# johanngerberding/voxelnet-pytorch

Hardware: AMD Instinct MI355X
Metric: point-clouds/sec fwd+bwd, KITTI car voxel grid, batch=2 (higher is better)
Workload: dtype bf16; 1 GPU; KITTI car config (voxel 0.2x0.2x0.4 m, grid 10x400x352, T=35), batch=2 per GPU, fwd+bwd train step (BASELINE configs[1]); global_batch=2, points_per_frame=19861, parallelism=dp1, launch_mode=eager+native-executor+one-call-step

## Files before the change

voxelnet-pytorch_amd/csrc/wgrad.hip:

```cpp
#include "common.h"

namespace {

constexpr uint32_t WG_OOB = 0xFFFFF000u;
constexpr uint32_t WG_MAX_WINDOW = 0xFFFFE000u;

struct WGParams {
    const char *src;
    const char *rows;
    float *dw;
    int64_t sB, sD, sH, sW;
    int64_t rB, rD, rH, rW;
    int32_t B, Ds, Hs, Ws, Dr, Hr, Wr;
    int32_t mulD, mulH, mulW, tmulD, tmulH, tmulW, padD, padH, padW;
    int32_t kD, kH, kW;
    int32_t C, N;
    int32_t x3;
    int32_t rows_per_chunk;
    int32_t tiles_k;
    uint32_t src_bytes, rows_bytes;
    const int64_t *row_list;
    int64_t n_rows;
    const int32_t *row_count;
    int32_t divD, divH, divW;
    float *part;
    int64_t part_stride;
};

typedef __attribute__((address_space(3))) void lds_void_t;
typedef __attribute__((ext_vector_type(4))) short s16x4_t;
typedef __attribute__((ext_vector_type(8))) short s16x8_t;

__device__ __forceinline__ void lds_dma16(__amdgpu_buffer_rsrc_t rsrc, char *lds_wave_base, uint32_t voffset,
                                          uint32_t soffset) {
    __builtin_amdgcn_raw_ptr_buffer_load_lds(rsrc, (lds_void_t *)lds_wave_base, 16, voffset, soffset, 0, 0);
}

template <int ROW_BYTES, bool F32, bool PS = false>
__device__ __forceinline__ int chunk_swz(int row) {
    if (PS) return (row & 1) | (((row >> 1) & 1) << 2) | (((row >> 3) & 1) << 3);
    if (F32) return (row & 3) << 2;
    if (ROW_BYTES == 128) return (((row >> 1) & 1) << 1) | (((row >> 3) & 1) << 2);
    return ((row & 3) << 1) | (((row >> 3) & 1) << 3);
}

template <int TN, int TK, bool F32, int TPB, int WKW = 2, bool PS = false>
__global__ void __launch_bounds__(128 * WKW, 2) k_wgrad(const WGParams p) {
    static_assert(!PS || F32, "split storage is fp32-sized");
    constexpr int NWV = 2 * WKW;
    constexpr int ESZ = F32 ? 4 : 2;
    constexpr int ROWS = F32 ? 32 : 64;
    constexpr int DN = 32 * TN, DK = 16 * WKW * TK;
    constexpr int RBN = DN * ESZ, RBK = DK * ESZ;
    constexpr int TILE_N = ROWS * RBN, TILE_K = ROWS * RBK;
    constexpr int STAGE = TILE_N + TPB * TILE_K;
    constexpr int IN = TILE_N / (1024 * NWV), IK = TILE_K / (1024 * NWV);
    static_assert(TILE_N % (1024 * NWV) == 0 && TILE_K % (1024 * NWV) == 0, "tile bytes per stage must split over the waves");
    constexpr int LPR_N = RBN / 16, LPR_K = RBK / 16;
    constexpr int TW = TPB + 1;
    extern __shared__ __attribute__((aligned(16))) char smem[];
    uint32_t *tbl = reinterpret_cast<uint32_t *>(smem + 2 * STAGE);

    const int lane = threadIdx.x & 63;
    const int wave = __builtin_amdgcn_readfirstlane(threadIdx.x >> 6);
    const int wn = wave / WKW, wk = wave % WKW;
    const int bx = blockIdx.x, by = blockIdx.y, tile = blockIdx.z, gx = gridDim.x;
    const int tn = tile / p.tiles_k, tk = tile - tn * p.tiles_k;
    const int n0 = tn * DN, k0 = tk * DK;
    const int tap0 = by * TPB;
    const int td = tap0 / (p.kH * p.kW), th = (tap0 / p.kW) % p.kH, tw0 = tap0 % p.kW;
    const bool list = p.row_list != nullptr;
    int64_t M = list ? p.n_rows : (int64_t)p.B * p.Dr * p.Hr * p.Wr;
    if (list && p.row_count) {
        const int64_t cnt = (int64_t)p.row_count[0];
        M = cnt < 0 ? 0 : (cnt < M ? cnt : M);
    }
    const bool dealt = list && p.row_count;
    int64_t rbeg = (int64_t)bx * p.rows_per_chunk;
    if (rbeg >= M && !dealt) return;
    int64_t rend = rbeg + p.rows_per_chunk;
    if (rend > M) rend = M;
    if (rend < rbeg) rend = rbeg;
    int nsteps = (int)((rend - rbeg + ROWS - 1) / ROWS);
    int64_t slab_stride = ROWS;
    if (dealt) {
        const int64_t nslabs = (M + ROWS - 1) / ROWS;
        nsteps = (int)(nslabs > bx ? (nslabs - bx + gx - 1) / gx : 0);
        rbeg = (int64_t)bx * ROWS;
        rend = M;
        slab_stride = (int64_t)gx * ROWS;
    }
    const int nstages = nsteps;

    const __amdgpu_buffer_rsrc_t rs_s = vn_uniform_rsrc(p.src, p.src_bytes);
    const __amdgpu_buffer_rsrc_t rs_r = vn_uniform_rsrc(p.rows, p.rows_bytes);

    int cb = 0, cd = 0, ch = 0, cw = 0;
    int cm32 = lane;
    const int rows_in_chunk = (int)(rend - rbeg);
    int tstep = 0;
    const uint32_t rBb = (uint32_t)(p.rB * ESZ), rDb = (uint32_t)(p.rD * ESZ), rHb = (uint32_t)(p.rH * ESZ), rWb = (uint32_t)(p.rW * ESZ);
    const uint32_t sBb = (uint32_t)(p.sB * ESZ), sDb = (uint32_t)(p.sD * ESZ), sHb = (uint32_t)(p.sH * ESZ), sWb = (uint32_t)(p.sW * ESZ);
    if (wave == 0 && !list) {
        int64_t t = rbeg + lane;
        cw = (int)(t % p.Wr); t /= p.Wr;
        ch = (int)(t % p.Hr); t /= p.Hr;
        cd = (int)(t % p.Dr);
        cb = (int)(t / p.Dr);
    }
    auto table_write = [&](int stage_idx) {
        const int step = stage_idx;
        uint32_t so[TPB], ro = WG_OOB;
#pragma unroll
        for (int j = 0; j < TPB; ++j) so[j] = WG_OOB;
        if (list) {
            const int64_t m = rbeg + (int64_t)step * slab_stride + lane;
            if (m < rend && lane < ROWS) {
                const int64_t *rc = p.row_list + m * 4;
                const int b = (int)rc[0];
                int sd = (int)rc[1] * p.mulD + td * p.tmulD - p.padD;
                int sh = (int)rc[2] * p.mulH + th * p.tmulH - p.padH;
                ro = (uint32_t)(m * p.rW * ESZ);
                const bool dh_ok = sd >= 0 && sh >= 0 && sd % p.divD == 0 && sh % p.divH == 0;
                sd /= p.divD; sh /= p.divH;
#pragma unroll
                for (int j = 0; j < TPB; ++j) {
                    int sw = (int)rc[3] * p.mulW + (tw0 + j) * p.tmulW - p.padW;
                    const bool ok = dh_ok && sw >= 0 && sw % p.divW == 0;
                    sw /= p.divW;
                    if (ok && sd < p.Ds && sh < p.Hs && sw < p.Ws)
                        so[j] = (uint32_t)(((int64_t)b * p.sB + (int64_t)sd * p.sD + (int64_t)sh * p.sH + (int64_t)sw * p.sW) * ESZ);
                }
            }
        } else {
            while (tstep < step) {
                cm32 += ROWS;
                cw += ROWS;
#pragma unroll
                for (int k = 0; k < 3; ++k) {
                    const bool wrap = cw >= p.Wr;
                    cw -= wrap ? p.Wr : 0;
                    ch += wrap ? 1 : 0;
                }
                while (cw >= p.Wr) { cw -= p.Wr; ++ch; }
                while (ch >= p.Hr) { ch -= p.Hr; ++cd; }
                while (cd >= p.Dr) { cd -= p.Dr; ++cb; }
                ++tstep;
            }
            if (cm32 < rows_in_chunk) {
                const int sd = cd * p.mulD + td * p.tmulD - p.padD;
                const int sh = ch * p.mulH + th * p.tmulH - p.padH;
                ro = (uint32_t)cb * rBb + (uint32_t)cd * rDb + (uint32_t)ch * rHb + (uint32_t)cw * rWb;
                if ((unsigned)sd < (unsigned)p.Ds && (unsigned)sh < (unsigned)p.Hs) {
                    const uint32_t base = (uint32_t)cb * sBb + (uint32_t)sd * sDb + (uint32_t)sh * sHb;
#pragma unroll
                    for (int j = 0; j < TPB; ++j) {
                        const int sw = cw * p.mulW + (tw0 + j) * p.tmulW - p.padW;
                        if ((unsigned)sw < (unsigned)p.Ws) so[j] = base + (uint32_t)sw * sWb;
                    }
                }
            }
        }
        uint32_t *e = tbl + ((stage_idx & 1) * 64 + lane) * TW;
#pragma unroll
        for (int j = 0; j < TPB; ++j) e[j] = so[j];
        e[TPB] = ro;
    };

    auto stage = [&](int sidx, int buf) {
        const uint32_t s_col = __builtin_amdgcn_readfirstlane((uint32_t)(k0 * ESZ));
        const uint32_t r_col = __builtin_amdgcn_readfirstlane((uint32_t)(n0 * ESZ));
        const uint32_t *t = tbl + (sidx & 1) * 64 * TW;
        char *ln = smem + buf * STAGE + wave * 1024;
#pragma unroll
        for (int i = 0; i < IN; ++i) {
            const int r = ((i * NWV + wave) * 1024) / RBN + lane / LPR_N;
            const int c = (lane % LPR_N) ^ chunk_swz<RBN, F32, PS>(r);
            const uint32_t ro = t[r * TW + TPB];
            const bool ok = ro != WG_OOB && (n0 + c * (16 / ESZ)) < p.N;
            lds_dma16(rs_r, ln + i * (1024 * NWV), ok ? ro + (uint32_t)c * 16u : WG_OOB, r_col);
        }
#pragma unroll
        for (int j = 0; j < TPB; ++j) {
            char *lk = smem + buf * STAGE + TILE_N + j * TILE_K + wave * 1024;
#pragma unroll
            for (int i = 0; i < IK; ++i) {
                const int r = ((i * NWV + wave) * 1024) / RBK + lane / LPR_K;
                const int c = (lane % LPR_K) ^ chunk_swz<RBK, F32, PS>(r);
                const uint32_t so = t[r * TW + j];
                const bool ok = so != WG_OOB && (k0 + c * (16 / ESZ)) < p.C;
                lds_dma16(rs_s, lk + i * (1024 * NWV), ok ? so + (uint32_t)c * 16u : WG_OOB, s_col);
            }
        }
    };

    f32x4_t acc[TPB][TN][TK];
#pragma unroll
    for (int t = 0; t < TPB; ++t)
#pragma unroll
        for (int i = 0; i < TN; ++i)
#pragma unroll
            for (int j = 0; j < TK; ++j) acc[t][i][j] = f32x4_t{0.f, 0.f, 0.f, 0.f};

    const int g = lane >> 4, q = (lane >> 2) & 3, pp = lane & 3;

    if (wave == 0 && nstages > 0) table_write(0);
    __syncthreads();
    if (nstages > 0) stage(0, 0);
    if (wave == 0 && nstages > 1) table_write(1);
    for (int s = 0; s < nstages; ++s) {
        const int buf = s & 1;
        asm volatile("s_waitcnt vmcnt(0)" ::: "memory");
        __syncthreads();
        if (s + 1 < nstages) stage(s + 1, buf ^ 1);
        if (wave == 0 && s + 2 < nstages) table_write(s + 2);
        const char *ln = smem + buf * STAGE;
        const char *lk0 = smem + buf * STAGE + TILE_N;
        if constexpr (PS) {
            typedef __attribute__((address_space(3))) s16x4_t lds_s16x4_t;
            static_assert(ROWS == 32, "one 32-site MFMA per stage");
            const int r0 = g * 8 + q, r1 = r0 + 4;
            const int sw0 = chunk_swz<RBN, true, true>(r0), sw1 = chunk_swz<RBN, true, true>(r1);
            const int pc = (pp >> 1) * 2, ph = (pp & 1) * 8;
            auto frag = [&](const char *tile, int row_bytes, int t16, int lo) {
                const int c16 = t16 * 4 + pc + lo;
                const char *p0 = tile + r0 * row_bytes + ((c16 ^ sw0) << 4) + ph;
                const char *p1 = tile + r1 * row_bytes + ((c16 ^ sw1) << 4) + ph;
                const s16x4_t v0 = __builtin_amdgcn_ds_read_tr16_b64_v4i16((lds_s16x4_t *)p0);
                const s16x4_t v1 = __builtin_amdgcn_ds_read_tr16_b64_v4i16((lds_s16x4_t *)p1);
                const s16x8_t t8 = __builtin_shufflevector(v0, v1, 0, 1, 2, 3, 4, 5, 6, 7);
                return __builtin_bit_cast(bf16x8_t, t8);
            };
            bf16x8_t ah[TN], al[TN];
#pragma unroll
            for (int i = 0; i < TN; ++i) {
                ah[i] = frag(ln, RBN, wn * TN + i, 0);
                al[i] = frag(ln, RBN, wn * TN + i, 1);
            }
#pragma unroll
            for (int t = 0; t < TPB; ++t)
#pragma unroll
                for (int j = 0; j < TK; ++j) {
                    const bf16x8_t bh = frag(lk0 + t * TILE_K, RBK, wk * TK + j, 0);
                    const bf16x8_t bl = frag(lk0 + t * TILE_K, RBK, wk * TK + j, 1);
#pragma unroll
                    for (int i = 0; i < TN; ++i) acc[t][i][j] = vn_mfma_x3(ah[i], al[i], bh, bl, acc[t][i][j]);
                }
        } else if constexpr (F32) {
            const int fc = lane & 15, kq = lane >> 4;
            if (p.x3) {
                static_assert(ROWS == 32, "eight sites per lane");
                bf16x8_t ah[TN], al[TN];
#pragma unroll
                for (int i = 0; i < TN; ++i) {
                    const int col = (wn * TN + i) * 16 + fc;
                    float v[8];
#pragma unroll
                    for (int ss = 0; ss < 8; ++ss) {
                        const int r = ss * 4 + kq;
                        v[ss] = *reinterpret_cast<const float *>(ln + r * RBN + ((((col >> 2) ^ chunk_swz<RBN, true>(r))) << 4) + (col & 3) * 4);
                    }
                    vn_split8(v, ah[i], al[i]);
                }
#pragma unroll
                for (int t = 0; t < TPB; ++t)
#pragma unroll
                    for (int j = 0; j < TK; ++j) {
                        const int col = (wk * TK + j) * 16 + fc;
                        float v[8];
#pragma unroll
                        for (int ss = 0; ss < 8; ++ss) {
                            const int r = ss * 4 + kq;
                            v[ss] = *reinterpret_cast<const float *>(lk0 + t * TILE_K + r * RBK + ((((col >> 2) ^ chunk_swz<RBK, true>(r))) << 4) + (col & 3) * 4);
                        }
                        bf16x8_t bh, bl;
                        vn_split8(v, bh, bl);
#pragma unroll
                        for (int i = 0; i < TN; ++i) acc[t][i][j] = vn_mfma_x3(ah[i], al[i], bh, bl, acc[t][i][j]);
                    }
            } else
#pragma unroll
            for (int ss = 0; ss < ROWS / 4; ++ss) {
                const int r = ss * 4 + kq;
                const int sw = chunk_swz<RBN, true>(r);
                float a[TN];
#pragma unroll
                for (int i = 0; i < TN; ++i) {
                    const int col = (wn * TN + i) * 16 + fc;
                    a[i] = *reinterpret_cast<const float *>(ln + r * RBN + ((((col >> 2) ^ sw)) << 4) + (col & 3) * 4);
                }
#pragma unroll
                for (int t = 0; t < TPB; ++t) {
                    float b[TK];
#pragma unroll
                    for (int j = 0; j < TK; ++j) {
                        const int col = (wk * TK + j) * 16 + fc;
                        b[j] = *reinterpret_cast<const float *>(lk0 + t * TILE_K + r * RBK + ((((col >> 2) ^ sw)) << 4) + (col & 3) * 4);
                    }
#pragma unroll
                    for (int i = 0; i < TN; ++i)
#pragma unroll
                        for (int j = 0; j < TK; ++j)
                            acc[t][i][j] = __builtin_amdgcn_mfma_f32_16x16x4f32(a[i], b[j], acc[t][i][j], 0, 0, 0);
                }
            }
        } else {
            typedef __attribute__((address_space(3))) s16x4_t lds_s16x4_t;
#pragma unroll
            for (int ks = 0; ks < 2; ++ks) {
                const int r0 = ks * 32 + g * 8 + q, r1 = r0 + 4;
                bf16x8_t a[TN];
#pragma unroll
                for (int i = 0; i < TN; ++i) {
                    const int col = (wn * TN + i) * 16 + pp * 4;
                    const int c16 = col >> 3, half = (col >> 2) & 1;
                    const char *p0 = ln + r0 * RBN + ((c16 ^ chunk_swz<RBN, false>(r0)) << 4) + half * 8;
                    const char *p1 = ln + r1 * RBN + ((c16 ^ chunk_swz<RBN, false>(r1)) << 4) + half * 8;
                    const s16x4_t lo = __builtin_amdgcn_ds_read_tr16_b64_v4i16((lds_s16x4_t *)p0);
                    const s16x4_t hi = __builtin_amdgcn_ds_read_tr16_b64_v4i16((lds_s16x4_t *)p1);
                    const s16x8_t t8 = __builtin_shufflevector(lo, hi, 0, 1, 2, 3, 4, 5, 6, 7);
                    a[i] = __builtin_bit_cast(bf16x8_t, t8);
                }
#pragma unroll
                for (int t = 0; t < TPB; ++t) {
                    bf16x8_t b[TK];
#pragma unroll
                    for (int j = 0; j < TK; ++j) {
                        const int col = (wk * TK + j) * 16 + pp * 4;
                        const int c16 = col >> 3, half = (col >> 2) & 1;
                        const char *p0 = lk0 + t * TILE_K + r0 * RBK + ((c16 ^ chunk_swz<RBK, false>(r0)) << 4) + half * 8;
                        const char *p1 = lk0 + t * TILE_K + r1 * RBK + ((c16 ^ chunk_swz<RBK, false>(r1)) << 4) + half * 8;
                        const s16x4_t lo = __builtin_amdgcn_ds_read_tr16_b64_v4i16((lds_s16x4_t *)p0);
                        const s16x4_t hi = __builtin_amdgcn_ds_read_tr16_b64_v4i16((lds_s16x4_t *)p1);
                        const s16x8_t t8 = __builtin_shufflevector(lo, hi, 0, 1, 2, 3, 4, 5, 6, 7);
                        b[j] = __builtin_bit_cast(bf16x8_t, t8);
                    }
#pragma unroll
                    for (int i = 0; i < TN; ++i)
#pragma unroll
                        for (int j = 0; j < TK; ++j)
                            acc[t][i][j] = __builtin_amdgcn_mfma_f32_16x16x32_bf16(a[i], b[j], acc[t][i][j], 0, 0, 0);
                }
            }
        }
    }

    float *dst = p.part ? p.part + (int64_t)bx * p.part_stride : p.dw;
#pragma unroll
    for (int t = 0; t < TPB; ++t)
#pragma unroll
        for (int i = 0; i < TN; ++i)
#pragma unroll
            for (int j = 0; j < TK; ++j) {
                const int k = k0 + (wk * TK + j) * 16 + (lane & 15);
#pragma unroll
                for (int e = 0; e < 4; ++e) {
                    const int n = n0 + (wn * TN + i) * 16 + (lane >> 4) * 4 + e;
                    if (n < p.N && k < p.C) {
                        float *q = dst + ((int64_t)(tap0 + t) * p.N + n) * p.C + k;
                        *q = p.part ? acc[t][i][j][e] : *q + acc[t][i][j][e];
                    }
                }
            }
}

__global__ void __launch_bounds__(256) k_wgrad_reduce(const float *__restrict__ part, int chunks, int64_t n4,
                                                      float *__restrict__ dw) {
    for (int64_t i = (int64_t)blockIdx.x * 256 + threadIdx.x; i < n4; i += (int64_t)gridDim.x * 256) {
        float4 s = make_float4(0.f, 0.f, 0.f, 0.f);
        for (int c = 0; c < chunks; ++c) {
            const float4 v = reinterpret_cast<const float4 *>(part)[(int64_t)c * n4 + i];
            s.x += v.x; s.y += v.y; s.z += v.z; s.w += v.w;
        }
        float4 d = reinterpret_cast<float4 *>(dw)[i];
        d.x += s.x; d.y += s.y; d.z += s.z; d.w += s.w;
        reinterpret_cast<float4 *>(dw)[i] = d;
    }
}

struct WPParams {
    const char *src, *rows;
    float *part;
    int64_t part_stride;
    int64_t sB, sD, sH, sW, rB, rD, rH, rW;
    int32_t B, Ds, Hs, Ws, Dr, Hr, Wr;
    int32_t mulD, padD, kD;
    int32_t C, N, tiles_k;
    int32_t tiles_x, tiles_y;
    int32_t tiles_per_chunk;
    uint32_t src_bytes, rows_bytes;
    uint32_t s_cb, s_part, r_cb, r_part;
};

template <int NH>
__global__ void __launch_bounds__(256 * NH, 2) k_wgrad_patch(const WPParams p) {
    constexpr int NWV = 4 * NH;
    constexpr int TH = 4, TW = 16, PH = TH + 2, LP = 32;
    constexpr int RB = 128;
    constexpr int RBN = 128 * NH;
    constexpr int TILE_N = 64 * RBN;
    constexpr int PATCH = PH * LP * RB;
    constexpr int STAGE = TILE_N + PATCH;
    constexpr int IN = TILE_N / (1024 * NWV);
    constexpr int RPI = 1024 / RBN, LPR = RBN / 16;
    constexpr int NPP = PH * 3;
    extern __shared__ __attribute__((aligned(16))) char smem[];
    const int lane = threadIdx.x & 63;
    const int wave = __builtin_amdgcn_readfirstlane(threadIdx.x >> 6);
    const int wn = wave >> 2, wk = wave & 3;
    const int tile = blockIdx.z;
    const int tn = tile / p.tiles_k, tk = tile - tn * p.tiles_k;
    const int n0 = tn * 64 * NH, k0 = tk * 64;
    const int kd = blockIdx.y;
    const int64_t ntiles = (int64_t)p.B * p.Dr * p.tiles_y * p.tiles_x;
    const int64_t tbeg = (int64_t)blockIdx.x * p.tiles_per_chunk;
    int64_t tend = tbeg + p.tiles_per_chunk;
    if (tend > ntiles) tend = ntiles;
    const int nst = (int)(tend - tbeg);

    const __amdgpu_buffer_rsrc_t rs_s = vn_uniform_rsrc(p.src, p.src_bytes);
    const __amdgpu_buffer_rsrc_t rs_r = vn_uniform_rsrc(p.rows, p.rows_bytes);
    const uint32_t s_col = (uint32_t)(k0 >> 3) * p.s_cb + p.s_part, r_col = (uint32_t)(n0 >> 3) * p.r_cb + p.r_part;

    int r_py[IN], r_px[IN];
    uint32_t r_dlt[IN], r_chunk[IN];
#pragma unroll
    for (int i = 0; i < IN; ++i) {
        const int r = (i * NWV + wave) * RPI + lane / LPR;
        const int c = (lane % LPR) ^ chunk_swz<RBN, false>(r);
        r_py[i] = r >> 4; r_px[i] = r & 15;
        r_dlt[i] = (uint32_t)((((int64_t)(r >> 4)) * p.rH + (int64_t)(r & 15) * p.rW) * 2) + (uint32_t)c * p.r_cb;
        r_chunk[i] = (n0 + c * 8) < p.N ? 1u : 0u;
    }
    constexpr int IPP = (NPP + NWV - 1) / NWV;
    int s_qy[IPP], s_qx[IPP];
    int32_t s_dlt[IPP];
    uint32_t s_ok[IPP], s_lds[IPP];
#pragma unroll
    for (int i = 0; i < IPP; ++i) {
        const int piece = i * NWV + wave;
        const int ql = piece / 3, cg = piece - ql * 3;
        const int qx = cg * 8 + lane / 8;
        const int prow = ql * LP + qx;
        const int c = (lane % 8) ^ chunk_swz<RB, false>(prow);
        s_qy[i] = ql - 1; s_qx[i] = qx - 1;
        s_dlt[i] = (int32_t)((((int64_t)(ql - 1)) * p.sH + (int64_t)(qx - 1) * p.sW) * 2) + c * (int32_t)p.s_cb;
        s_ok[i] = (piece < NPP && qx < TW + 2 && (k0 + c * 8) < p.C) ? 1u : 0u;
        s_lds[i] = (uint32_t)((ql * LP + cg * 8) * RB);
    }
    int tx, ty, td, tb;
    {
        int64_t t = tbeg;
        tx = (int)(t % p.tiles_x); t /= p.tiles_x;
        ty = (int)(t % p.tiles_y); t /= p.tiles_y;
        td = (int)(t % p.Dr);
        tb = (int)(t / p.Dr);
    }
    auto stage = [&](int buf) {
        const int y0 = ty * TH, x0 = tx * TW;
        const int sd = td * p.mulD + kd - p.padD;
        const bool plane_ok = (unsigned)sd < (unsigned)p.Ds;
        const uint32_t rbase = (uint32_t)(((int64_t)tb * p.rB + (int64_t)td * p.rD + (int64_t)y0 * p.rH + (int64_t)x0 * p.rW) * 2);
        const uint32_t sbase = (uint32_t)(((int64_t)tb * p.sB + (int64_t)sd * p.sD + (int64_t)y0 * p.sH + (int64_t)x0 * p.sW) * 2);
        char *ln = smem + buf * STAGE + wave * 1024;
#pragma unroll
        for (int i = 0; i < IN; ++i) {
            const bool ok = plane_ok && r_chunk[i] && y0 + r_py[i] < p.Hr && x0 + r_px[i] < p.Wr;
            lds_dma16(rs_r, ln + i * (1024 * NWV), ok ? rbase + r_dlt[i] : WG_OOB, r_col);
        }
        char *lp = smem + buf * STAGE + TILE_N;
#pragma unroll
        for (int i = 0; i < IPP; ++i) {
            if (i * NWV + wave >= NPP) break;
            const bool ok = plane_ok && s_ok[i] && (unsigned)(y0 + s_qy[i]) < (unsigned)p.Hs &&
                            (unsigned)(x0 + s_qx[i]) < (unsigned)p.Ws;
            lds_dma16(rs_s, lp + s_lds[i], ok ? sbase + (uint32_t)s_dlt[i] : WG_OOB, s_col);
        }
        if (++tx == p.tiles_x) {
            tx = 0;
            if (++ty == p.tiles_y) {
                ty = 0;
                if (++td == p.Dr) { td = 0; ++tb; }
            }
        }
    };

    f32x4_t acc[9][4];
#pragma unroll
    for (int t = 0; t < 9; ++t)
#pragma unroll
        for (int i = 0; i < 4; ++i) acc[t][i] = f32x4_t{0.f, 0.f, 0.f, 0.f};

    const int g = lane >> 4, q = (lane >> 2) & 3, pp = lane & 3;
    typedef __attribute__((address_space(3))) s16x4_t lds_s16x4_t;
    int aoff[4][2];
#pragma unroll
    for (int i = 0; i < 4; ++i) {
        const int col = (wn * 4 + i) * 16 + pp * 4, c16 = col >> 3, half = (col >> 2) & 1;
        const int r0 = g * 8 + q;
        aoff[i][0] = r0 * RBN + ((c16 ^ chunk_swz<RBN, false>(r0)) << 4) + half * 8;
        aoff[i][1] = (r0 + 4) * RBN + ((c16 ^ chunk_swz<RBN, false>(r0 + 4)) << 4) + half * 8;
    }
    int boff[3][2];
#pragma unroll
    for (int tw = 0; tw < 3; ++tw)
#pragma unroll
        for (int wq = 0; wq < 2; ++wq) {
            const int colw = (g & 1) * 8 + q + tw + 4 * wq;
            const int sw = chunk_swz<RB, false>(colw);
            const int col = wk * 16 + pp * 4, c16 = col >> 3, half = (col >> 2) & 1;
            boff[tw][wq] = ((g >> 1) * LP + colw) * RB + ((c16 ^ sw) << 4) + half * 8;
        }

    stage(0);
    for (int s = 0; s < nst; ++s) {
        const int buf = s & 1;
        asm volatile("s_waitcnt vmcnt(0)" ::: "memory");
        __syncthreads();
        if (s + 1 < nst) stage(buf ^ 1);
        const char *ln = smem + buf * STAGE;
        const char *lp = ln + TILE_N;
#pragma unroll
        for (int ks = 0; ks < 2; ++ks) {
            bf16x8_t a[4];
#pragma unroll
            for (int i = 0; i < 4; ++i) {
                const s16x4_t lo = __builtin_amdgcn_ds_read_tr16_b64_v4i16((lds_s16x4_t *)(ln + ks * 32 * RBN + aoff[i][0]));
                const s16x4_t hi = __builtin_amdgcn_ds_read_tr16_b64_v4i16((lds_s16x4_t *)(ln + ks * 32 * RBN + aoff[i][1]));
                a[i] = __builtin_bit_cast(bf16x8_t, __builtin_shufflevector(lo, hi, 0, 1, 2, 3, 4, 5, 6, 7));
            }
#pragma unroll
            for (int t = 0; t < 9; ++t) {
                const int th = t / 3, tw = t % 3;
                const char *lt = lp + (ks * 2 + th) * LP * RB;
                const s16x4_t lo = __builtin_amdgcn_ds_read_tr16_b64_v4i16((lds_s16x4_t *)(lt + boff[tw][0]));
                const s16x4_t hi = __builtin_amdgcn_ds_read_tr16_b64_v4i16((lds_s16x4_t *)(lt + boff[tw][1]));
                const bf16x8_t bq = __builtin_bit_cast(bf16x8_t, __builtin_shufflevector(lo, hi, 0, 1, 2, 3, 4, 5, 6, 7));
#pragma unroll
                for (int i = 0; i < 4; ++i) acc[t][i] = __builtin_amdgcn_mfma_f32_16x16x32_bf16(bq, a[i], acc[t][i], 0, 0, 0);
            }
        }
    }
    float *dst = p.part + (int64_t)blockIdx.x * p.part_stride;
#pragma unroll
    for (int t = 0; t < 9; ++t)
#pragma unroll
        for (int i = 0; i < 4; ++i) {
            const int k = k0 + wk * 16 + (lane >> 4) * 4;
            const int n = n0 + (wn * 4 + i) * 16 + (lane & 15);
            if (n < p.N && k < p.C)
                *reinterpret_cast<f32x4_t *>(dst + ((int64_t)(kd * 9 + t) * p.N + n) * p.C + k) = acc[t][i];
        }
}

template <int TN, int TK, bool F32, int TPB, int WKW = 2, bool PS = false>
int launch_wgrad(const WGParams &p, dim3 grid, hipStream_t st) {
    constexpr int DN = 32 * TN, DK = 16 * WKW * TK;
    constexpr size_t lds = 2u * 64u * (DN + TPB * DK) * 2u + 2u * 64u * (TPB + 1) * 4u;
    static const hipError_t attr = hipFuncSetAttribute(reinterpret_cast<const void *>(&k_wgrad<TN, TK, F32, TPB, WKW, PS>),
                                                       hipFuncAttributeMaxDynamicSharedMemorySize, (int)lds);
    if (attr != hipSuccess) return (int)attr;
    k_wgrad<TN, TK, F32, TPB, WKW, PS><<<grid, 128 * WKW, lds, st>>>(p);
    VN_LAUNCH_STATUS();
    return VN_OK;
}

}

static int wgrad_impl(const void *src, const void *rows, float *dw_packed, const vnConv *g, int32_t split,
                      const int64_t *row_list, int64_t n_rows, void *workspace, size_t workspace_bytes, vnStream stream,
                      int32_t *chunks_out = nullptr, const int32_t *row_count = nullptr, int split_pass = -1);

struct WGPlan {
    bool tri, n128, k128;
    int tiles_n, tiles_k, groups;
    int64_t chunks;
    int64_t dw_elems;
};
static WGPlan wgrad_plan(const vnConv *g, int32_t split, int64_t M) {
    WGPlan w{};
    const bool f32 = g->dtype != VN_BF16;
    const int taps = g->kD * g->kH * g->kW;
    w.tri = !f32 && !split && g->kW == 3 && g->Cr <= 64;
    w.n128 = !w.tri && g->Cr > 64;
    w.k128 = g->Cs > 64;
    w.tiles_n = (int)vn_ceil_div(g->Cr, w.n128 ? 128 : 64);
    w.tiles_k = (int)vn_ceil_div(g->Cs, w.k128 ? 128 : 64);
    w.groups = w.tri ? taps / 3 : taps;
    w.dw_elems = (int64_t)taps * g->Cr * g->Cs;
    static const int knob = vn_knob("VN_WG_BLOCKS", 0);
    const int target = knob > 0 ? knob : ((g->dtype == VN_F32X3 || g->dtype == VN_F32X3S) ? 384 : 256);
    int64_t chunks = target / ((int64_t)w.groups * w.tiles_n * w.tiles_k);
    const int64_t slabs = vn_ceil_div(M, 64);
    if (chunks > slabs / 10) chunks = slabs / 10;
    if (chunks > 256) chunks = 256;
    if (chunks < 1) chunks = 1;
    w.chunks = chunks;
    return w;
}

struct WPPlan {
    bool ok;
    int nh;
    int tiles_x, tiles_y, tiles_n, tiles_k;
    int64_t ntiles, chunks;
};
static int wgrad_patch_enabled() {
    static const int v = vn_knob("VN_WGRAD_PATCH", 1);
    return v;
}
static WPPlan wgrad_patch_plan(const vnConv *g, int32_t split, bool list) {
    WPPlan w{};
    if (!wgrad_patch_enabled() || list || split || g->dtype != VN_BF16) return w;
    if (g->kH != 3 || g->kW != 3 || g->mulH != 1 || g->mulW != 1 || g->tmulH != 1 || g->tmulW != 1 || g->padH != 1 ||
        g->padW != 1 || g->tmulD != 1 || g->divD != 1 || g->divH != 1 || g->divW != 1)
        return w;
    if (g->Hs != g->Hr || g->Ws != g->Wr) return w;
    if (g->Cr > 64 || g->Hr < 128 || g->Wr < 128 || g->Cs > 64) return w;
    w.nh = 1;
    w.tiles_x = (int)vn_ceil_div(g->Wr, 16);
    w.tiles_y = (int)vn_ceil_div(g->Hr, 4);
    w.tiles_n = (int)vn_ceil_div(g->Cr, 64 * w.nh);
    w.tiles_k = (int)vn_ceil_div(g->Cs, 64);
    w.ntiles = (int64_t)g->B * g->Dr * w.tiles_y * w.tiles_x;
    static const int ptarget = vn_knob("VN_WGP_BLOCKS", 256);
    int64_t chunks = ptarget / ((int64_t)g->kD * w.tiles_n * w.tiles_k);
    const int64_t min_stages = 8;
    if (chunks > w.ntiles / min_stages) chunks = w.ntiles / min_stages;
    if (chunks > 256) chunks = 256;
    if (chunks < 1) chunks = 1;
    w.chunks = chunks;
    w.ok = true;
    return w;
}

extern "C" size_t vn_conv_wgrad_workspace_bytes(const vnConv *g, int32_t split, int64_t n_rows) {
    if (!g || g->B <= 0 || g->Dr <= 0 || g->Hr <= 0 || g->Wr <= 0 || g->Cs <= 0 || g->Cr <= 0) return 0;
    if (g->kD < 1 || g->kH < 1 || g->kW < 1) return 0;
    const int64_t M = n_rows > 0 ? n_rows : (int64_t)g->B * g->Dr * g->Hr * g->Wr;
    const WGPlan w = wgrad_plan(g, split, M);
    int64_t chunks = w.chunks;
    const WPPlan wp = wgrad_patch_plan(g, split, n_rows > 0);
    if (wp.ok && wp.chunks > chunks) chunks = wp.chunks;
    return (size_t)chunks * (size_t)w.dw_elems * sizeof(float);
}

extern "C" int32_t vn_conv_wgrad_plan_id(const vnConv *g, int32_t split, int64_t n_rows) {
    if (!g || g->B <= 0 || g->Dr <= 0 || g->Hr <= 0 || g->Wr <= 0 || g->Cs <= 0 || g->Cr <= 0) return -1;
    const int64_t M = n_rows > 0 ? n_rows : (int64_t)g->B * g->Dr * g->Hr * g->Wr;
    const WPPlan wp = wgrad_patch_plan(g, split, n_rows > 0);
    if (wp.ok) return 200;
    const WGPlan w = wgrad_plan(g, split, M);
    if (w.tri) return 1000 + 10 * 2 + (w.k128 ? 4 : 2);
    return 10 * (w.n128 ? 4 : 2) + (w.k128 ? 4 : 2);
}

extern "C" int vn_conv_wgrad(const void *src, const void *rows, float *dw_packed, const vnConv *g, int32_t split,
                             void *workspace, size_t workspace_bytes, vnStream stream) {
    return wgrad_impl(src, rows, dw_packed, g, split, nullptr, 0, workspace, workspace_bytes, stream);
}

extern "C" int vn_conv_wgrad_partials(const void *src, const void *rows, const vnConv *g, int32_t split,
                                      const int64_t *row_list, int64_t n_rows, void *workspace, size_t workspace_bytes,
                                      int32_t *chunks, vnStream stream) {
    VN_CHECK_ARG(chunks && workspace && (row_list || n_rows == 0));
    if (row_list && n_rows == 0) {
        const size_t bytes = (size_t)g->kD * g->kH * g->kW * g->Cr * g->Cs * sizeof(float);
        if (workspace_bytes < bytes) return VN_EWORKSPACE;
        VN_HIP(hipMemsetAsync(workspace, 0, bytes, vn_stream(stream)));
        *chunks = 1;
        return VN_OK;
    }
    return wgrad_impl(src, rows, static_cast<float *>(workspace), g, row_list ? 0 : split, row_list, n_rows, workspace,
                      workspace_bytes, stream, chunks);
}

extern "C" int vn_conv_wgrad_partials_counted(const void *src, const void *rows, const vnConv *g, const int64_t *row_list,
                                              int64_t row_cap, const int32_t *row_count, void *workspace,
                                              size_t workspace_bytes, int32_t *chunks, vnStream stream) {
    VN_CHECK_ARG(chunks && workspace && row_list && row_count && row_cap > 0);
    return wgrad_impl(src, rows, static_cast<float *>(workspace), g, 0, row_list, row_cap, workspace, workspace_bytes, stream,
                      chunks, row_count);
}

extern "C" int vn_conv_wgrad_partials_split_pass(const void *src, const void *rows, const vnConv *g, int32_t pass, void *workspace,
                                                 size_t workspace_bytes, int32_t *chunks, vnStream stream) {
    VN_CHECK_ARG(g && chunks && workspace && pass >= 0 && pass <= 2 && g->dtype == VN_F32X3S);
    if ((g->Cs & 7) || (g->Cr & 7)) return VN_EUNSUPPORTED;
    vnConv b = *g;
    b.dtype = VN_BF16;
    b.src_sB *= 2; b.src_sD *= 2; b.src_sH *= 2; b.src_sW *= 2;
    b.out_sB *= 2; b.out_sD *= 2; b.out_sH *= 2; b.out_sW *= 2;
    return wgrad_impl(src, rows, static_cast<float *>(workspace), &b, 0, nullptr, 0, workspace, workspace_bytes, stream, chunks,
                      nullptr, pass);
}

extern "C" int vn_conv_wgrad_rows(const void *src, const void *rows, float *dw_packed, const vnConv *g,
                                  const int64_t *row_list, int64_t n_rows, void *workspace, size_t workspace_bytes,
                                  vnStream stream) {
    if (!row_list || n_rows < 0) return VN_EINVAL;
    if (n_rows == 0) return VN_OK;
    return wgrad_impl(src, rows, dw_packed, g, 0, row_list, n_rows, workspace, workspace_bytes, stream);
}

static int wgrad_impl(const void *src, const void *rows, float *dw_packed, const vnConv *g, int32_t split,
                      const int64_t *row_list, int64_t n_rows, void *workspace, size_t workspace_bytes, vnStream stream,
                      int32_t *chunks_out, const int32_t *row_count, int split_pass) {
    const bool partial_only = chunks_out != nullptr;
    if (partial_only) dw_packed = static_cast<float *>(workspace);
    VN_CHECK_ARG(src && rows && dw_packed && g);
    VN_CHECK_ARG(g->B > 0 && g->Ds > 0 && g->Hs > 0 && g->Ws > 0 && g->Dr > 0 && g->Hr > 0 && g->Wr > 0);
    VN_CHECK_ARG(g->kD >= 1 && g->kH >= 1 && g->kW >= 1 && g->kD * g->kH * g->kW <= 65535);
    if (!row_list && (g->divD != 1 || g->divH != 1 || g->divW != 1)) return VN_EUNSUPPORTED;
    if (g->divD < 1 || g->divH < 1 || g->divW < 1) return VN_EINVAL;
    VN_CHECK_ARG(g->dtype == VN_BF16 || ((g->dtype == VN_F32 || g->dtype == VN_F32X3 || g->dtype == VN_F32X3S) && !split));
    const bool ps = g->dtype == VN_F32X3S;
    if (ps && ((g->Cs & 15) || (g->Cr & 15) || ((g->src_sB | g->src_sD | g->src_sH | g->src_sW | g->out_sB | g->out_sD | g->out_sH | g->out_sW) & 7)))
        return VN_EUNSUPPORTED;
    const bool f32 = g->dtype != VN_BF16;
    const int esz = f32 ? 4 : 2, al = 16 / esz - 1;
    if (g->Cs <= 0 || (g->Cs & al) || g->Cr <= 0 || (g->Cr & al)) return VN_EUNSUPPORTED;
    if (((g->src_sB | g->src_sD | g->src_sH | g->src_sW) & al) != 0) return VN_EUNSUPPORTED;
    if (((g->out_sB | g->out_sD | g->out_sH | g->out_sW) & al) != 0) return VN_EUNSUPPORTED;
    if ((reinterpret_cast<uintptr_t>(src) & 15) || (reinterpret_cast<uintptr_t>(rows) & 15)) return VN_EUNSUPPORTED;

    WGParams p{};
    p.src = static_cast<const char *>(src);
    p.rows = static_cast<const char *>(rows);
    p.dw = dw_packed;
    p.sB = g->src_sB; p.sD = g->src_sD; p.sH = g->src_sH; p.sW = g->src_sW;
    p.rB = g->out_sB; p.rD = g->out_sD; p.rH = g->out_sH; p.rW = g->out_sW;
    p.B = g->B; p.Ds = g->Ds; p.Hs = g->Hs; p.Ws = g->Ws; p.Dr = g->Dr; p.Hr = g->Hr; p.Wr = g->Wr;
    p.mulD = g->mulD; p.mulH = g->mulH; p.mulW = g->mulW;
    p.tmulD = g->tmulD; p.tmulH = g->tmulH; p.tmulW = g->tmulW;
    p.padD = g->padD; p.padH = g->padH; p.padW = g->padW;
    p.kD = g->kD; p.kH = g->kH; p.kW = g->kW;
    p.C = g->Cs; p.N = g->Cr;
    if (split) return VN_EUNSUPPORTED;
    p.x3 = g->dtype == VN_F32X3 || ps;
    const int wmul = split_pass >= 0 ? 2 : 1;
    const int64_t sbytes = ((int64_t)(g->B - 1) * g->src_sB + (int64_t)(g->Ds - 1) * g->src_sD +
                            (int64_t)(g->Hs - 1) * g->src_sH + (int64_t)(g->Ws - 1) * g->src_sW + wmul * g->Cs) * esz;
    const int64_t rbytes = row_list ? ((n_rows - 1) * g->out_sW + wmul * g->Cr) * esz
                                    : ((int64_t)(g->B - 1) * g->out_sB + (int64_t)(g->Dr - 1) * g->out_sD +
                                       (int64_t)(g->Hr - 1) * g->out_sH + (int64_t)(g->Wr - 1) * g->out_sW + wmul * g->Cr) * esz;
    if (sbytes > (int64_t)WG_MAX_WINDOW || rbytes > (int64_t)WG_MAX_WINDOW) return VN_EUNSUPPORTED;
    p.src_bytes = (uint32_t)sbytes;
    p.rows_bytes = (uint32_t)rbytes;

    const int64_t M = row_list ? n_rows : (int64_t)g->B * g->Dr * g->Hr * g->Wr;
    const WGPlan w = wgrad_plan(g, split, M);
    const bool tri = w.tri, n128 = w.n128, k128 = w.k128;
    const int tiles_n = w.tiles_n, tiles_k = w.tiles_k, groups = w.groups;
    p.tiles_k = tiles_k;
    p.row_list = row_list;
    p.n_rows = n_rows;
    p.row_count = row_list ? row_count : nullptr;
    p.divD = g->divD; p.divH = g->divH; p.divW = g->divW;
    const WPPlan wp = wgrad_patch_plan(g, split, row_list != nullptr);
    if (wp.ok && workspace && !(reinterpret_cast<uintptr_t>(workspace) & 15) && !(w.dw_elems & 3) &&
        (int64_t)(workspace_bytes / ((size_t)w.dw_elems * sizeof(float))) >= 1) {
        int64_t pchunks = wp.chunks;
        const int64_t room = (int64_t)(workspace_bytes / ((size_t)w.dw_elems * sizeof(float)));
        if (pchunks > room) pchunks = room;
        WPParams q{};
        q.src = p.src; q.rows = p.rows;
        q.part = static_cast<float *>(workspace);
        q.part_stride = w.dw_elems;
        q.sB = p.sB; q.sD = p.sD; q.sH = p.sH; q.sW = p.sW;
        q.rB = p.rB; q.rD = p.rD; q.rH = p.rH; q.rW = p.rW;
        q.B = p.B; q.Ds = p.Ds; q.Hs = p.Hs; q.Ws = p.Ws; q.Dr = p.Dr; q.Hr = p.Hr; q.Wr = p.Wr;
        q.mulD = p.mulD; q.padD = p.padD; q.kD = p.kD;
        q.C = p.C; q.N = p.N; q.tiles_k = wp.tiles_k;
        q.tiles_x = wp.tiles_x; q.tiles_y = wp.tiles_y;
        q.tiles_per_chunk = (int32_t)vn_ceil_div(wp.ntiles, pchunks);
        pchunks = vn_ceil_div(wp.ntiles, q.tiles_per_chunk);
        q.src_bytes = p.src_bytes; q.rows_bytes = p.rows_bytes;
        q.s_cb = q.r_cb = split_pass >= 0 ? 32u : 16u;
        q.s_part = split_pass == 1 ? 16u : 0u;
        q.r_part = split_pass == 2 ? 16u : 0u;
        hipStream_t pst = vn_stream(stream);
        const dim3 pgrid((unsigned)pchunks, (unsigned)g->kD, (unsigned)(wp.tiles_n * wp.tiles_k));
        {
            constexpr size_t lds = 2 * (64 * 128 + 6 * 32 * 128);
            static const hipError_t attr = hipFuncSetAttribute(reinterpret_cast<const void *>(&k_wgrad_patch<1>),
                                                               hipFuncAttributeMaxDynamicSharedMemorySize, (int)lds);
            if (attr != hipSuccess) return (int)attr;
            k_wgrad_patch<1><<<pgrid, 256, lds, pst>>>(q);
        }
        VN_LAUNCH_STATUS();
        if (partial_only) {
            *chunks_out = (int32_t)pchunks;
        } else {
            const int64_t n4 = w.dw_elems / 4;
            int64_t blocks = vn_ceil_div(n4, 256);
            if (blocks > 2048) blocks = 2048;
            k_wgrad_reduce<<<(unsigned)blocks, 256, 0, pst>>>(q.part, (int)pchunks, n4, dw_packed);
            VN_LAUNCH_STATUS();
        }
        return VN_OK;
    }
    if (split_pass >= 0) return VN_EUNSUPPORTED;
    int64_t chunks = w.chunks;
    const int64_t room = workspace ? (int64_t)(workspace_bytes / ((size_t)w.dw_elems * sizeof(float))) : 0;
    if (chunks > room) chunks = room;
    if ((w.dw_elems & 3) || (reinterpret_cast<uintptr_t>(workspace) & 15) || (reinterpret_cast<uintptr_t>(dw_packed) & 15))
        chunks = 1;
    if (chunks < 2) chunks = 1;
    int64_t rpc = vn_ceil_div(vn_ceil_div(M, chunks), 64) * 64;
    if (rpc < 64) rpc = 64;
    if (rpc > (1 << 30)) return VN_EUNSUPPORTED;
    p.rows_per_chunk = (int32_t)rpc;
    chunks = vn_ceil_div(M, rpc);
    p.part = (chunks > 1 || partial_only) ? static_cast<float *>(workspace) : nullptr;
    if (partial_only) {
        if (!workspace || (int64_t)(workspace_bytes / ((size_t)w.dw_elems * sizeof(float))) < chunks) return VN_EWORKSPACE;
        *chunks_out = (int32_t)chunks;
    }
    p.part_stride = w.dw_elems;
    dim3 grid((unsigned)chunks, (unsigned)groups, (unsigned)(tiles_n * tiles_k));
    hipStream_t st = vn_stream(stream);
    int rc;
    if (tri) rc = k128 ? launch_wgrad<2, 2, false, 3, 4>(p, grid, st) : launch_wgrad<2, 1, false, 3, 4>(p, grid, st);
    else if (ps) {
        if (n128 && k128) rc = launch_wgrad<4, 2, true, 1, 4, true>(p, grid, st);
        else if (n128) rc = launch_wgrad<4, 1, true, 1, 4, true>(p, grid, st);
        else if (k128) rc = launch_wgrad<2, 2, true, 1, 4, true>(p, grid, st);
        else rc = launch_wgrad<2, 1, true, 1, 4, true>(p, grid, st);
    } else if (f32 && p.x3) {
        if (n128 && k128) rc = launch_wgrad<4, 2, true, 1, 4>(p, grid, st);
        else if (n128) rc = launch_wgrad<4, 1, true, 1, 4>(p, grid, st);
        else if (k128) rc = launch_wgrad<2, 2, true, 1, 4>(p, grid, st);
        else rc = launch_wgrad<2, 1, true, 1, 4>(p, grid, st);
    } else if (f32) {
        if (n128 && k128) rc = launch_wgrad<4, 4, true, 1>(p, grid, st);
        else if (n128) rc = launch_wgrad<4, 2, true, 1>(p, grid, st);
        else if (k128) rc = launch_wgrad<2, 4, true, 1>(p, grid, st);
        else rc = launch_wgrad<2, 2, true, 1>(p, grid, st);
    } else {
        if (n128 && k128) rc = launch_wgrad<4, 2, false, 1, 4>(p, grid, st);
        else if (n128) rc = launch_wgrad<4, 1, false, 1, 4>(p, grid, st);
        else if (k128) rc = launch_wgrad<2, 2, false, 1, 4>(p, grid, st);
        else rc = launch_wgrad<2, 1, false, 1, 4>(p, grid, st);
    }
    if (rc != VN_OK) return rc;
    if (chunks > 1 && !partial_only) {
        const int64_t n4 = w.dw_elems / 4;
        int64_t blocks = vn_ceil_div(n4, 256);
        if (blocks > 2048) blocks = 2048;
        k_wgrad_reduce<<<(unsigned)blocks, 256, 0, st>>>(p.part, (int)chunks, n4, dw_packed);
        VN_LAUNCH_STATUS();
    }
    return VN_OK;
}
```

Measured before the change: 570.2 point-clouds/s.

## Skip out-of-range depth planes and bin-pack kD taps into roles in wgrad patch kernel

The patch weight-gradient kernel now iterates only over depth output planes whose source plane is valid for each kD tap, instead of staging zero-filled tiles for out-of-range planes. A host-side first-fit packer groups kD taps with fewer valid planes into shared grid 'roles', so one block handles several taps in sequence. This shrinks the grid's y dimension and aims to balance work across blocks. It adds per-tap accumulator flushes and prologue overhead, and the packed tables cap kD at 8.

```diff
diff --git a/voxelnet-pytorch_amd/csrc/wgrad.hip b/voxelnet-pytorch_amd/csrc/wgrad.hip
--- a/voxelnet-pytorch_amd/csrc/wgrad.hip
+++ b/voxelnet-pytorch_amd/csrc/wgrad.hip
@@ -390,6 +390,9 @@
     int32_t tiles_per_chunk;
     uint32_t src_bytes, rows_bytes;
     uint32_t s_cb, s_part, r_cb, r_part;
+    int32_t role_tab;
+    uint32_t role_kds;
+    uint64_t role_beg;
 };
 
 template <int NH>
@@ -411,12 +414,14 @@
     const int tile = blockIdx.z;
     const int tn = tile / p.tiles_k, tk = tile - tn * p.tiles_k;
     const int n0 = tn * 64 * NH, k0 = tk * 64;
-    const int kd = blockIdx.y;
-    const int64_t ntiles = (int64_t)p.B * p.Dr * p.tiles_y * p.tiles_x;
+    const int role = blockIdx.y;
+    int ri = p.role_tab ? (int)((p.role_beg >> (4 * role)) & 15) : role;
+    const int rend = p.role_tab ? (int)((p.role_beg >> (4 * (role + 1))) & 15) : role + 1;
+    const int64_t plane = (int64_t)p.tiles_y * p.tiles_x;
+    const int64_t ntiles = (int64_t)p.B * p.Dr * plane;
     const int64_t tbeg = (int64_t)blockIdx.x * p.tiles_per_chunk;
     int64_t tend = tbeg + p.tiles_per_chunk;
     if (tend > ntiles) tend = ntiles;
-    const int nst = (int)(tend - tbeg);
 
     const __amdgpu_buffer_rsrc_t rs_s = vn_uniform_rsrc(p.src, p.src_bytes);
     const __amdgpu_buffer_rsrc_t rs_r = vn_uniform_rsrc(p.rows, p.rows_bytes);
@@ -448,48 +453,55 @@
         s_ok[i] = (piece < NPP && qx < TW + 2 && (k0 + c * 8) < p.C) ? 1u : 0u;
         s_lds[i] = (uint32_t)((ql * LP + cg * 8) * RB);
     }
-    int tx, ty, td, tb;
-    {
+    int kd = 0, tlo = 0, thi = 0, tx = 0, ty = 0, td = 0, tb = 0;
+    int64_t tnext = tend;
+    auto begin_kd = [&](int k) {
+        kd = k;
+        tlo = p.Dr; thi = 0;
+        for (int d = 0; d < p.Dr; ++d)
+            if ((unsigned)(d * p.mulD + kd - p.padD) < (unsigned)p.Ds) {
+                if (d < tlo) tlo = d;
+                thi = d + 1;
+            }
         int64_t t = tbeg;
         tx = (int)(t % p.tiles_x); t /= p.tiles_x;
         ty = (int)(t % p.tiles_y); t /= p.tiles_y;
         td = (int)(t % p.Dr);
         tb = (int)(t / p.Dr);
-    }
+        if (td < tlo) { td = tlo; ty = tx = 0; }
+        else if (td >= thi) { td = tlo; ty = tx = 0; ++tb; }
+        tnext = tlo < thi ? (((int64_t)tb * p.Dr + td) * p.tiles_y + ty) * p.tiles_x + tx : tend;
+    };
     auto stage = [&](int buf) {
         const int y0 = ty * TH, x0 = tx * TW;
         const int sd = td * p.mulD + kd - p.padD;
-        const bool plane_ok = (unsigned)sd < (unsigned)p.Ds;
         const uint32_t rbase = (uint32_t)(((int64_t)tb * p.rB + (int64_t)td * p.rD + (int64_t)y0 * p.rH + (int64_t)x0 * p.rW) * 2);
         const uint32_t sbase = (uint32_t)(((int64_t)tb * p.sB + (int64_t)sd * p.sD + (int64_t)y0 * p.sH + (int64_t)x0 * p.sW) * 2);
         char *ln = smem + buf * STAGE + wave * 1024;
 #pragma unroll
         for (int i = 0; i < IN; ++i) {
-            const bool ok = plane_ok && r_chunk[i] && y0 + r_py[i] < p.Hr && x0 + r_px[i] < p.Wr;
+            const bool ok = r_chunk[i] && y0 + r_py[i] < p.Hr && x0 + r_px[i] < p.Wr;
             lds_dma16(rs_r, ln + i * (1024 * NWV), ok ? rbase + r_dlt[i] : WG_OOB, r_col);
         }
         char *lp = smem + buf * STAGE + TILE_N;
 #pragma unroll
         for (int i = 0; i < IPP; ++i) {
             if (i * NWV + wave >= NPP) break;
-            const bool ok = plane_ok && s_ok[i] && (unsigned)(y0 + s_qy[i]) < (unsigned)p.Hs &&
-                            (unsigned)(x0 + s_qx[i]) < (unsigned)p.Ws;
+            const bool ok = s_ok[i] && (unsigned)(y0 + s_qy[i]) < (unsigned)p.Hs && (unsigned)(x0 + s_qx[i]) < (unsigned)p.Ws;
             lds_dma16(rs_s, lp + s_lds[i], ok ? sbase + (uint32_t)s_dlt[i] : WG_OOB, s_col);
         }
+        ++tnext;
         if (++tx == p.tiles_x) {
             tx = 0;
             if (++ty == p.tiles_y) {
                 ty = 0;
-                if (++td == p.Dr) { td = 0; ++tb; }
+                if (++td == thi) { td = tlo; ++tb; tnext += (int64_t)(p.Dr - thi + tlo) * plane; }
             }
         }
     };
 
     f32x4_t acc[9][4];
-#pragma unroll
-    for (int t = 0; t < 9; ++t)
-#pragma unroll
-        for (int i = 0; i < 4; ++i) acc[t][i] = f32x4_t{0.f, 0.f, 0.f, 0.f};
+    auto kd_of = [&](int i) { return p.role_tab ? (int)((p.role_kds >> (4 * i)) & 15) : i; };
 
     const int g = lane >> 4, q = (lane >> 2) & 3, pp = lane & 3;
     typedef __attribute__((address_space(3))) s16x4_t lds_s16x4_t;
@@ -512,45 +524,64 @@
             boff[tw][wq] = ((g >> 1) * LP + colw) * RB + ((c16 ^ sw) << 4) + half * 8;
         }
 
-    stage(0);
-    for (int s = 0; s < nst; ++s) {
-        const int buf = s & 1;
-        asm volatile("s_waitcnt vmcnt(0)" ::: "memory");
-        __syncthreads();
-        if (s + 1 < nst) stage(buf ^ 1);
-        const char *ln = smem + buf * STAGE;
-        const char *lp = ln + TILE_N;
-#pragma unroll
-        for (int ks = 0; ks < 2; ++ks) {
-            bf16x8_t a[4];
+    float *const dst = p.part + (int64_t)blockIdx.x * p.part_stride;
+    int buf = 0;
+    begin_kd(kd_of(ri));
+    bool staged = tnext < tend;
+    if (staged) stage(0);
+    for (;;) {
+#pragma unroll
+        for (int t = 0; t < 9; ++t)
+#pragma unroll
+            for (int i = 0; i < 4; ++i) acc[t][i] = f32x4_t{0.f, 0.f, 0.f, 0.f};
+        while (staged) {
+            asm volatile("s_waitcnt vmcnt(0)" ::: "memory");
+            __syncthreads();
+            const bool more = tnext < tend;
+            if (more) stage(buf ^ 1);
+            const char *ln = smem + buf * STAGE;
+            const char *lp = ln + TILE_N;
+#pragma unroll
+            for (int ks = 0; ks < 2; ++ks) {
+                bf16x8_t a[4];
+#pragma unroll
+                for (int i = 0; i < 4; ++i) {
+                    const s16x4_t lo = __builtin_amdgcn_ds_read_tr16_b64_v4i16((lds_s16x4_t *)(ln + ks * 32 * RBN + aoff[i][0]));
+                    const s16x4_t hi = __builtin_amdgcn_ds_read_tr16_b64_v4i16((lds_s16x4_t *)(ln + ks * 32 * RBN + aoff[i][1]));
+                    a[i] = __builtin_bit_cast(bf16x8_t, __builtin_shufflevector(lo, hi, 0, 1, 2, 3, 4, 5, 6, 7));
+                }
+#pragma unroll
+                for (int t = 0; t < 9; ++t) {
+                    const int th = t / 3, tw = t % 3;
+                    const char *lt = lp + (ks * 2 + th) * LP * RB;
+                    const s16x4_t lo = __builtin_amdgcn_ds_read_tr16_b64_v4i16((lds_s16x4_t *)(lt + boff[tw][0]));
+                    const s16x4_t hi = __builtin_amdgcn_ds_read_tr16_b64_v4i16((lds_s16x4_t *)(lt + boff[tw][1]));
+                    const bf16x8_t bq = __builtin_bit_cast(bf16x8_t, __builtin_shufflevector(lo, hi, 0, 1, 2, 3, 4, 5, 6, 7));
+#pragma unroll
+                    for (int i = 0; i < 4; ++i) acc[t][i] = __builtin_amdgcn_mfma_f32_16x16x32_bf16(bq, a[i], acc[t][i], 0, 0, 0);
+                }
+            }
+            buf ^= 1;
+            staged = more;
+        }
+        const int kd_done = kd;
+        const bool last = ++ri == rend;
+        if (!last) {
+            begin_kd(kd_of(ri));
+            staged = tnext < tend;
+            if (staged) stage(buf);
+        }
+#pragma unroll
+        for (int t = 0; t < 9; ++t)
 #pragma unroll
             for (int i = 0; i < 4; ++i) {
-                const s16x4_t lo = __builtin_amdgcn_ds_read_tr16_b64_v4i16((lds_s16x4_t *)(ln + ks * 32 * RBN + aoff[i][0]));
-                const s16x4_t hi = __builtin_amdgcn_ds_read_tr16_b64_v4i16((lds_s16x4_t *)(ln + ks * 32 * RBN + aoff[i][1]));
-                a[i] = __builtin_bit_cast(bf16x8_t, __builtin_shufflevector(lo, hi, 0, 1, 2, 3, 4, 5, 6, 7));
-            }
-#pragma unroll
-            for (int t = 0; t < 9; ++t) {
-                const int th = t / 3, tw = t % 3;
-                const char *lt = lp + (ks * 2 + th) * LP * RB;
-                const s16x4_t lo = __builtin_amdgcn_ds_read_tr16_b64_v4i16((lds_s16x4_t *)(lt + boff[tw][0]));
-                const s16x4_t hi = __builtin_amdgcn_ds_read_tr16_b64_v4i16((lds_s16x4_t *)(lt + boff[tw][1]));
-                const bf16x8_t bq = __builtin_bit_cast(bf16x8_t, __builtin_shufflevector(lo, hi, 0, 1, 2, 3, 4, 5, 6, 7));
-#pragma unroll
-                for (int i = 0; i < 4; ++i) acc[t][i] = __builtin_amdgcn_mfma_f32_16x16x32_bf16(bq, a[i], acc[t][i], 0, 0, 0);
-            }
-        }
-    }
-    float *dst = p.part + (int64_t)blockIdx.x * p.part_stride;
-#pragma unroll
-    for (int t = 0; t < 9; ++t)
-#pragma unroll
-        for (int i = 0; i < 4; ++i) {
-            const int k = k0 + wk * 16 + (lane >> 4) * 4;
-            const int n = n0 + (wn * 4 + i) * 16 + (lane & 15);
-            if (n < p.N && k < p.C)
-                *reinterpret_cast<f32x4_t *>(dst + ((int64_t)(kd * 9 + t) * p.N + n) * p.C + k) = acc[t][i];
-        }
+                const int k = k0 + wk * 16 + (lane >> 4) * 4;
+                const int n = n0 + (wn * 4 + i) * 16 + (lane & 15);
+                if (n < p.N && k < p.C)
+                    *reinterpret_cast<f32x4_t *>(dst + ((int64_t)(kd_done * 9 + t) * p.N + n) * p.C + k) = acc[t][i];
+            }
+        if (last) break;
+    }
 }
 
 template <int TN, int TK, bool F32, int TPB, int WKW = 2, bool PS = false>
@@ -604,7 +635,41 @@
     int nh;
     int tiles_x, tiles_y, tiles_n, tiles_k;
     int64_t ntiles, chunks;
+    int nroles, role_tab;
+    uint32_t role_kds;
+    uint64_t role_beg;
 };
+static void wgrad_patch_roles(const vnConv *g, WPPlan &w) {
+    w.nroles = g->kD; w.role_tab = 0; w.role_kds = 0; w.role_beg = 0;
+    if (g->kD > 8) return;
+    int cnt[8], order[8], bin[8], load[8], maxc = 0, nb = 0;
+    for (int kd = 0; kd < g->kD; ++kd) {
+        cnt[kd] = 0;
+        for (int td = 0; td < g->Dr; ++td) cnt[kd] += (unsigned)(td * g->mulD + kd - g->padD) < (unsigned)g->Ds;
+        if (cnt[kd] > maxc) maxc = cnt[kd];
+        int i = kd;
+        for (; i > 0 && cnt[order[i - 1]] < cnt[kd]; --i) order[i] = order[i - 1];
+        order[i] = kd;
+    }
+    for (int i = 0; i < g->kD; ++i) {
+        int b = 0;
+        while (b < nb && load[b] + cnt[order[i]] > maxc) ++b;
+        if (b == nb) load[nb++] = 0;
+        load[b] += cnt[order[i]];
+        bin[order[i]] = b;
+    }
+    if (nb == g->kD)
+        for (int kd = 0; kd < g->kD; ++kd) bin[kd] = kd;
+    int n = 0;
+    for (int b = 0; b < nb; ++b) {
+        w.role_beg |= (uint64_t)n << (4 * b);
+        for (int kd = 0; kd < g->kD; ++kd)
+            if (bin[kd] == b) w.role_kds |= (uint32_t)kd << (4 * n++);
+    }
+    w.role_beg |= (uint64_t)n << (4 * nb);
+    w.nroles = nb;
+    w.role_tab = 1;
+}
 static int wgrad_patch_enabled() {
     static const int v = vn_knob("VN_WGRAD_PATCH", 1);
     return v;
@@ -624,6 +689,7 @@
     w.tiles_k = (int)vn_ceil_div(g->Cs, 64);
     w.ntiles = (int64_t)g->B * g->Dr * w.tiles_y * w.tiles_x;
     static const int ptarget = vn_knob("VN_WGP_BLOCKS", 256);
+    wgrad_patch_roles(g, w);
     int64_t chunks = ptarget / ((int64_t)g->kD * w.tiles_n * w.tiles_k);
     const int64_t min_stages = 8;
     if (chunks > w.ntiles / min_stages) chunks = w.ntiles / min_stages;
@@ -779,8 +845,9 @@
         q.s_cb = q.r_cb = split_pass >= 0 ? 32u : 16u;
         q.s_part = split_pass == 1 ? 16u : 0u;
         q.r_part = split_pass == 2 ? 16u : 0u;
+        q.role_tab = wp.role_tab; q.role_kds = wp.role_kds; q.role_beg = wp.role_beg;
         hipStream_t pst = vn_stream(stream);
-        const dim3 pgrid((unsigned)pchunks, (unsigned)g->kD, (unsigned)(wp.tiles_n * wp.tiles_k));
+        const dim3 pgrid((unsigned)pchunks, (unsigned)wp.nroles, (unsigned)(wp.tiles_n * wp.tiles_k));
         {
             constexpr size_t lds = 2 * (64 * 128 + 6 * 32 * 128);
             static const hipError_t attr = hipFuncSetAttribute(reinterpret_cast<const void *>(&k_wgrad_patch<1>),
```

Result: no change. 570.4 point-clouds/s (median of 2 runs) (+0.0%).
